# codename0og/codename-rvc-fork-3

Measured on AMD Instinct MI355X. Metric: 48 kHz audio samples/sec end-to-end VC, higher is better.
Workload: dtype f32 (vocoder ResBlock convs and upsamplers, HuBERT, RMVPE's U-Net convs: fp32 operands as exact bf16x3 splits on the bf16 matrix cores -- six products of order <= 2^-16 per multiply-add, fp32 accumulate; everything else fp32 / fp64)

## Files before the change

codename-rvc-fork-3_amd/csrc/decoder.hip:

```cpp
#include <stdlib.h>

#include "decoder.h"

namespace rvc {


constexpr int CARRY_CHUNK = 4096;
__global__ void __launch_bounds__(256)
nsf_carry_kernel(const float *__restrict__ f0, int64_t T, float sr, float upp, float *__restrict__ carry) {
    __shared__ double pre[CARRY_CHUNK];
    __shared__ double part[257];
    __shared__ double cum_s;
    constexpr int SEG = CARRY_CHUNK / 256;
    const int64_t b = blockIdx.x;
    const float *f = f0 + b * T;
    float *c = carry + b * T;
    if (threadIdx.x == 0) {
        c[0] = 0.f;
        cum_s = 0.0;
    }
    for (int64_t base = 0; base + 1 < T; base += CARRY_CHUNK) {
        const int n = (int)((T - 1 - base) < CARRY_CHUNK ? (T - 1 - base) : CARRY_CHUNK);
        for (int i = threadIdx.x; i < n; i += 256) {
            const float last = __fmul_rn(__fdiv_rn(f[base + i], sr), upp);
// ... 409 lines not shown
                if (out->wx.upload(frags)) return 1;
            }
        }
    }
    if (c_in != c_out && !as_bf16 && k >= 7 && winobf_enabled() && winobf_supported(c_in, c_out, k, 1)) {
        std::vector<uint16_t> frags;
        winobf_pack_host(w->data.data(), c_out, c_in, k, &frags);
        if (out->wx.upload(frags)) return 1;
    }
    if (bias) {
        if (need(d, prefix + ".bias", &b, {c_out})) return 1;
        if (out->b.upload(b->data)) return 1;
    }
    out->c_in = c_in; out->c_out = c_out; out->k = k;
    return 0;
}
}

extern "C" int rvc_decoder_create(const rvc_decoder_config *cfg, rvc_decoder **out) {
    if (!cfg || !out) return fail("rvc_decoder_create: null pointer");
    if (cfg->kind != RVC_DEC_NSF && cfg->kind != RVC_DEC_MRF && cfg->kind != RVC_DEC_REFINE)
        return fail("rvc_decoder_create: unknown decoder kind %d", cfg->kind);
    if (cfg->n_ups < 1 || cfg->n_ups > 8) return fail("rvc_decoder_create: n_ups out of range");
    if (cfg->n_res_kernels < 1 || cfg->n_res_kernels > 4 || cfg->n_res_dilations < 1 || cfg->n_res_dilations > 4)
        return fail("rvc_decoder_create: resblock configuration out of range");
    if (cfg->weight_storage != 0 && cfg->weight_storage != 1) return fail("rvc_decoder_create: weight_storage must be 0 (fp32) or 1 (bf16)");
    if (cfg->weight_storage == 1 && cfg->kind == RVC_DEC_REFINE)
        return fail("rvc_decoder_create: bf16 weight storage is built for the NSF / MRF decoders (BASELINE cfg 4), not RefineGAN");
    if (cfg->in_channels % 8 || cfg->upsample_initial_channel % (32 << cfg->n_ups))
        return fail("rvc_decoder_create: channel counts must keep every stage a multiple of 32");
    rvc_decoder *d = new rvc_decoder();
    d->cfg = *cfg;
    d->upp = 1;
    for (int i = 0; i < cfg->n_ups; ++i) d->upp *= cfg->upsample_rates[i];
    if (d->upp > 1024) { delete d; return fail("rvc_decoder_create: prod(upsample_rates) > 1024"); }
    d->dim = cfg->kind == RVC_DEC_MRF ? 9 : 1;
    *out = d;
    return 0;
}

extern "C" int rvc_decoder_set_arithmetic(rvc_decoder *dec, int mode) {
    if (!dec) return fail("rvc_decoder_set_arithmetic: null decoder");
    if (mode != 0 && mode != 1) return fail("rvc_decoder_set_arithmetic: mode must be 0 (exact) or 1 (fp16 pairs), got %d", mode);
    if (dec->finalized) return fail("rvc_decoder_set_arithmetic: decoder already finalized (the tap slabs are packed at finalize)");
    if (mode == 1 && dec->cfg.weight_storage == 1)
        return fail("rvc_decoder_set_arithmetic: fp16 pairs are for fp32 taps; a weight_storage = 1 handle's bf16 taps already cost three products");
    dec->arithmetic = mode;
    return 0;
}

extern "C" int rvc_decoder_set_tensor(rvc_decoder *dec, const char *name, const float *data_host, const int64_t *shape,
                                      int ndim) {
    if (!dec || !name || !data_host || !shape || ndim < 1 || ndim > 4) return fail("rvc_decoder_set_tensor: bad argument");
    if (dec->finalized) return fail("rvc_decoder_set_tensor: decoder already finalized");
    HostTensor t;
    t.shape.assign(shape, shape + ndim);
    const int64_t n = t.numel();
    if (n <= 0) return fail("rvc_decoder_set_tensor: empty tensor '%s'", name);
    t.data.assign(data_host, data_host + n);
    dec->host[name] = std::move(t);
    return 0;
}

extern "C" int rvc_decoder_finalize(rvc_decoder *d) {
    if (!d) return fail("rvc_decoder_finalize: null decoder");
    if (d->finalized) return 0;
    if (d->cfg.kind == RVC_DEC_REFINE) {
        if (refine_finalize(d)) return 1;
        d->host.clear();
        d->finalized = true;
        return 0;
    }
    const rvc_decoder_config &c = d->cfg;
    const bool mrf = c.kind == RVC_DEC_MRF;
    const HostTensor *t;
    if (need(d, "m_source.l_linear.weight", &t, {1, d->dim})) return 1;
    for (int h = 0; h < d->dim; ++h) d->lin_w[h] = t->data[h];
    if (need(d, "m_source.l_linear.bias", &t, {1})) return 1;
    d->lin_b = t->data[0];
    const int c0 = c.upsample_initial_channel;
    if (build_conv(d, "conv_pre", c0, c.in_channels, 7, true, &d->pre)) return 1;
    if (need(d, "cond.weight", &t, {c0, c.gin_channels, 1})) return 1;
    if (d->cond_w.upload(t->data)) return 1;
    if (need(d, "cond.bias", &t, {c0})) return 1;
    if (d->cond_b.upload(t->data)) return 1;
    d->stages.clear();
    d->stages.resize(c.n_ups);
    for (int i = 0; i < c.n_ups; ++i) {
        Stage &s = d->stages[i];
        s.c_in = c0 >> i;
        s.c_out = c0 >> (i + 1);
        s.rate = c.upsample_rates[i];
        s.ksize = c.upsample_kernel_sizes[i];
        s.pad = (s.rate % 2 == 0) ? (s.ksize - s.rate) / 2 : s.rate / 2 + s.rate % 2;
        s.opad = s.rate % 2;
        s.taps = (s.ksize + s.rate - 1) / s.rate;
        if (s.taps > 2) return fail("decoder: upsample kernel %d with rate %d needs %d polyphase taps (max 2)", s.ksize, s.rate, s.taps);
        if (s.taps < 2) s.taps = 2;
        int stride_f0 = 1;
        for (int j = i + 1; j < c.n_ups; ++j) stride_f0 *= c.upsample_rates[j];
        s.nc_stride = stride_f0;
        s.nc_k = stride_f0 == 1 ? 1 : stride_f0 * 2 - stride_f0 % 2;
        s.nc_pad = stride_f0 == 1 ? 0 : (s.nc_k - stride_f0) / 2;
        s.vk = (s.rate - 1) * s.nc_stride + s.nc_k;
        s.vk_rows = (s.vk + 7) / 8 * 8;
        s.S = (int64_t)s.rate * s.nc_stride;
        s.P = (int64_t)s.pad * s.nc_stride + s.nc_pad;
        static const int nc_sep_env = knob("RVC_NC_SEPARATE", 1);
        const bool nc_separate = nc_sep_env && s.vk_rows * 2 >= s.c_in;
        if (nc_separate) {
            s.nc_rows = (s.nc_k + 7) / 8 * 8;
            s.vk = 0;
            s.vk_rows = 0;
        }

        const std::string up = (mrf ? "upsamples." : "ups.") + std::to_string(i);
        const std::string nc = "noise_convs." + std::to_string(i);
        const HostTensor *uw, *ub, *nw, *nb;
        if (need(d, up + ".weight", &uw, {s.c_in, s.c_out, s.ksize})) return 1;
        if (need(d, up + ".bias", &ub, {s.c_out})) return 1;
        if (need(d, nc + ".weight", &nw, {s.c_out, 1, s.nc_k})) return 1;
        if (need(d, nc + ".bias", &nb, {s.c_out})) return 1;
        const int ctot = s.c_in + s.vk_rows;
        const int m_total = s.rate * s.c_out;
        s.interleave = s.rate % 2 == 0;
        auto mrow = [&](int ph, int co) { return s.interleave ? co * s.rate + ph : ph * s.c_out + co; };
        std::vector<float> packed((size_t)s.taps * ctot * m_total, 0.f);
        for (int tp = 0; tp < s.taps; ++tp) {
            const int j = s.taps - 1 - tp;
            for (int ci = 0; ci < s.c_in; ++ci)
                for (int ph = 0; ph < s.rate; ++ph) {
                    const int kk = ph + j * s.rate;
                    if (kk >= s.ksize) continue;
                    for (int co = 0; co < s.c_out; ++co)
                        packed[((size_t)tp * ctot + ci) * m_total + mrow(ph, co)] =
                            uw->data[((size_t)ci * s.c_out + co) * s.ksize + kk];
                }
        }
        const int tp0 = s.taps - 1;
        for (int kq = 0; kq < s.vk; ++kq)
            for (int ph = 0; ph < s.rate; ++ph) {
                const int k = kq - ph * s.nc_stride;
                if (k < 0 || k >= s.nc_k) continue;
                for (int co = 0; co < s.c_out; ++co)
                    packed[((size_t)tp0 * ctot + s.c_in + kq) * m_total + mrow(ph, co)] = nw->data[(size_t)co * s.nc_k + k];
            }
        if (s.w.upload(packed)) return 1;
        std::vector<float> bias(s.c_out);
        for (int co = 0; co < s.c_out; ++co) bias[co] = ub->data[co] + nb->data[co];
        {
            static const int ups_bf = knob("RVC_UPS_BF", 1);
            const int k_n = s.nc_rows > 0 ? 0 : s.nc_k;
            const int vk = upsbf_fold_noise(k_n) ? (s.rate - 1) * s.nc_stride + k_n : 0;
            if (ups_bf && s.opad == 0 && s.rate * s.c_out >= 128 && upsbf_supported(s.c_in, s.c_out, s.rate, s.ksize, vk)) {
                std::vector<uint16_t> frags;
                upsbf_pack_host(uw->data.data(), k_n ? nw->data.data() : nullptr, bias.data(), s.c_in, s.c_out, s.rate, s.ksize, vk, k_n, s.nc_stride, &frags);
                if (s.wub.upload(frags)) return 1;
                s.ub_vk = vk;
            }
        }
        if (s.nc_rows) {
            std::vector<float> ncw((size_t)s.nc_rows * s.c_out, 0.f);
            for (int k = 0; k < s.nc_k; ++k)
                for (int co = 0; co < s.c_out; ++co) ncw[(size_t)k * s.c_out + co] = nw->data[(size_t)co * s.nc_k + k];
            if (s.nc_w.upload(ncw)) return 1;
        }
        if (s.b.upload(bias)) return 1;

        const int nb_ = c.n_res_kernels * c.n_res_dilations;
        s.c1 = std::vector<ConvW>(nb_);
        s.c2 = std::vector<ConvW>(nb_);
        s.pair = std::vector<DevBuf16>(nb_);
        for (int m = 0; m < c.n_res_kernels; ++m)
            for (int j = 0; j < c.n_res_dilations; ++j) {
                std::string p1, p2;
                if (mrf) {
                    const std::string base = "mrfs." + std::to_string(i) + "." + std::to_string(m) + ".layers." + std::to_string(j);
                    p1 = base + ".conv1";
                    p2 = base + ".conv2";
                } else {
                    const std::string base = "resblocks." + std::to_string(i * c.n_res_kernels + m);
                    p1 = base + ".convs1." + std::to_string(j);
                    p2 = base + ".convs2." + std::to_string(j);
                }
                const int k = c.res_kernel_sizes[m];
                const bool b16 = c.weight_storage == 1 && (k == 3 || k == 7 || k == 11);
                if (build_conv(d, p1, s.c_out, s.c_out, k, true, &s.c1[m * c.n_res_dilations + j], b16)) return 1;
                if (build_conv(d, p2, s.c_out, s.c_out, k, true, &s.c2[m * c.n_res_dilations + j], b16)) return 1;
                const int nts = b16 ? 1 : 3;
                if (resblock_bf_enabled() && resblock_bf_supported(s.c_out, k, 1) && resblock_bf_preferred(s.c_out, k, nts)) {
                    const HostTensor *w1, *w2;
                    if (need(d, p1 + ".weight", &w1, {s.c_out, s.c_out, k}) || need(d, p2 + ".weight", &w2, {s.c_out, s.c_out, k})) return 1;
                    std::vector<uint16_t> frags;
                    resblock_bf_pack_host(w1->data.data(), w2->data.data(), s.c_out, k, &frags, nts);
                    s.pair_splits = nts;
                    if (s.pair[m * c.n_res_dilations + j].upload(frags)) return 1;
                }
            }
    }
    d->post_cin = c0 >> c.n_ups;
    if (need(d, "conv_post.weight", &t, {1, d->post_cin, 7})) return 1;
    if (d->post_w.upload(t->data)) return 1;
    d->post_b = 0.f;
    if (mrf) {
        if (need(d, "conv_post.bias", &t, {1})) return 1;
        d->post_b = t->data[0];
    }
    d->host.clear();
    d->finalized = true;
    return 0;
}

extern "C" int rvc_decoder_destroy(rvc_decoder *dec) {
    delete dec;
    return 0;
}

extern "C" int rvc_decoder_upp(const rvc_decoder *dec) { return dec ? dec->upp : 0; }

namespace {
struct Carve {
    size_t off = 0;
    size_t take(size_t bytes) { size_t o = off; off += align_up(bytes, 256); return o; }
};
struct Layout {
    size_t har, carry, biasp, V, p1, p2, wraps, buf[2 + 2 * (MAX_BRANCH_LANES + 1)], total;
    int n_buf;
    int64_t max_cl;
};
constexpr int64_t BRANCH_PARALLEL_MAX_ELEMS = (int64_t)3 * 256 * 128 * 256;
int branch_lanes_wanted(const rvc_decoder *d) {
    const int nk = d->cfg.n_res_kernels, want = d->branch_parallel.load(std::memory_order_relaxed);
    const int most = nk - 1 < MAX_BRANCH_LANES ? nk - 1 : MAX_BRANCH_LANES;
    return want < 0 || want > most ? most : want;
}
Layout make_layout(const rvc_decoder *d, int batch, int64_t T, int64_t Tw) {
    Layout l;
    Carve c;
    const int64_t L = Tw * d->upp;
    l.har = c.take((size_t)batch * L * 4);
    l.carry = c.take((size_t)batch * T * 4);
    l.biasp = c.take((size_t)batch * d->cfg.upsample_initial_channel * 4);
    int64_t len = Tw, max_cl = (int64_t)std::max(d->cfg.upsample_initial_channel, d->cfg.in_channels) * Tw, max_v = 0;
    for (const Stage &s : d->stages) {
        const int64_t nq = len + 1;
        max_v = std::max<int64_t>(max_v, (int64_t)s.vk_rows * nq);
        len = (len - 1) * s.rate - 2 * s.pad + s.ksize + s.opad;
        max_v = std::max<int64_t>(max_v, (int64_t)s.nc_rows * len);
        max_cl = std::max<int64_t>(max_cl, (int64_t)s.c_out * len);
    }
    l.V = c.take((size_t)batch * max_v * 4);
    const size_t scan = d->dim > 1 ? (size_t)batch * d->dim * T : 0;
    l.p1 = c.take(scan * 8);
    l.p2 = c.take(scan * 8);
    l.wraps = c.take(scan * 4);
    l.n_buf = 2 + 2 * (branch_lanes_wanted(d) + 1);
    for (int i = 0; i < l.n_buf; ++i) l.buf[i] = c.take((size_t)batch * max_cl * 4);
    l.total = c.off;
    l.max_cl = max_cl;
    return l;
}
}

extern "C" int rvc_decoder_workspace_bytes(const rvc_decoder *dec, int batch, int64_t n_frames, size_t *bytes) {
    if (!dec || !bytes || batch <= 0 || n_frames <= 0) return fail("rvc_decoder_workspace_bytes: bad argument");
    if (!dec->finalized) return fail("rvc_decoder_workspace_bytes: decoder not finalized");
    *bytes = dec->cfg.kind == RVC_DEC_REFINE ? refine_workspace_bytes(dec, batch, n_frames) : make_layout(dec, batch, n_frames, n_frames).total;
    return 0;
}

extern "C" int rvc_decoder_set_tap(rvc_decoder *dec, int stage, float *tap_dev) {
    if (!dec) return fail("rvc_decoder_set_tap: null decoder");
    dec->tap_stage = tap_dev ? stage : -2;
    dec->tap_dev = tap_dev;
    return 0;
}

int rvc::BranchLanes::create(int n) {
    n_side = n;
    for (int i = 0; i < n; ++i) RVC_HIP(hipStreamCreateWithFlags(&side[i], hipStreamNonBlocking));
    RVC_HIP(hipEventCreateWithFlags(&fork, hipEventDisableTiming));
    for (int i = 0; i <= MAX_BRANCH_LANES; ++i) RVC_HIP(hipEventCreateWithFlags(&last[i], hipEventDisableTiming));
    return 0;
}
rvc::BranchLanes::~BranchLanes() {
    for (int i = 0; i < n_side; ++i) if (side[i]) { (void)hipStreamSynchronize(side[i]); (void)hipStreamDestroy(side[i]); }
    if (fork) (void)hipEventDestroy(fork);
    for (int i = 0; i <= MAX_BRANCH_LANES; ++i) if (last[i]) (void)hipEventDestroy(last[i]);
}

namespace {
int lanes_for(rvc_decoder *d, hipStream_t stream, int n_side, BranchLanes **out) {
    std::lock_guard<std::mutex> g(d->lanes_mu);
    BranchLanes *&l = d->lanes[stream];
    if (l && l->n_side != n_side) { delete l; l = nullptr; }
    if (!l) {
        l = new BranchLanes();
        if (l->create(n_side)) { delete l; l = nullptr; return 1; }
    }
    *out = l;
    return 0;
}
}

extern "C" int rvc_decoder_set_branch_parallel(rvc_decoder *dec, int side_streams) {
    if (!dec) return fail("rvc_decoder_set_branch_parallel: null decoder");
    dec->branch_parallel.store(side_streams, std::memory_order_relaxed);
// ... 292 lines not shown
```

codename-rvc-fork-3_amd/csrc/upsbf.hip:

```cpp
#include <stdlib.h>

#include <algorithm>
#include <mutex>
#include <type_traits>
#include <vector>

#include "conv.h"

namespace rvc {

constexpr int UB_NTH = 512;
constexpr int UB_CK = 64;

struct UbParams {
    const float *x = nullptr;
    const float *har = nullptr;
    const void *u = nullptr;
    const float *bias = nullptr;
    float *y = nullptr;
    int64_t L_in = 0, L_out = 0, Lh = 0;
    int c_in = 0, c_out = 0;
    int n_xchunks = 0;
    int vk = 0;
    int S = 0, P = 0;
    int pad = 0;
    float slope = 0.1f;
    int n_mblk = 0, col_tiles = 0, n_tiles = 0, per_xcd = 0;
};

template <int R, int MB>
struct UbGeom {
    static constexpr int RB_T = MB / 32;
    static constexpr int RBW = RB_T >= 4 ? RB_T / 4 : 1;
    static constexpr int CG = RB_T >= 4 ? 1 : 4 / RB_T;
    static constexpr int N1 = 64 * CG;
    static constexpr int W = N1 * R;
    static constexpr int CPB = (MB - 1) / R + 2;
    static constexpr int KS = UB_CK / 16;
    static constexpr int NGC = 2 * KS;
    static constexpr int PA = 4;
    static constexpr int ROWB = 6 * UB_CK + 16;
    static constexpr int XROWS = N1 + 1;
    static constexpr int X_BYTES = (XROWS + 1) * ROWB;
    static constexpr int RC32 = (XROWS + 31) / 32;
    static constexpr int NIT = (UB_CK / 8) * RC32 / 4;
    static constexpr int IO_FLOATS = CPB * W;
    static constexpr int IO_BYTES = IO_FLOATS * 4 + 16;
    static constexpr int LDS_BYTES = 2 * X_BYTES + IO_BYTES;
    static constexpr int GROUP_BYTES = RB_T * 3 * 1024;
    static_assert(MB == 64 || MB == 128 || MB == 256, "GEMM rows per tile");
    static_assert(R >= 1 && R <= MB, "a channel's phases span at most two m-blocks");
    static_assert((UB_CK / 8) * RC32 % 4 == 0, "the items must divide over the four stager waves");
    static_assert(NGC % PA == 0 && KS % PA == 0, "a chunk's groups must be whole turns of the tap ring");
    static_assert(LDS_BYTES <= 163840, "LDS budget");
};

template <int R, int MB>
__global__ void __launch_bounds__(UB_NTH) __attribute__((amdgpu_waves_per_eu(2, 2)))
upsbf_kernel(const UbParams p) {
    using GM = UbGeom<R, MB>;
    constexpr int RB_T = GM::RB_T, RBW = GM::RBW, N1 = GM::N1, W = GM::W, KS = GM::KS, NGC = GM::NGC, PA = GM::PA, ROWB = GM::ROWB;
    constexpr int NIT = GM::NIT, CK = UB_CK;

    extern __shared__ __attribute__((aligned(16))) unsigned char ub_smem[];
    unsigned char *const xs = ub_smem;
    float *const io_lds = reinterpret_cast<float *>(ub_smem + 2 * GM::X_BYTES);

    const int tid = threadIdx.x, lane = tid & 63;
    const int wave = __builtin_amdgcn_readfirstlane(tid >> 6);
    const int half = lane >> 5, l31 = lane & 31;
    const int64_t L_in = p.L_in, L_out = p.L_out;
    const int nxc = p.n_xchunks, ncht = nxc + (p.vk > 0 ? 1 : 0);
    const int ngt = nxc * NGC + (p.vk > 0 ? KS : 0);
    const int n_mblk = p.n_mblk;
    const int m_total = p.c_out * R;

    const int xcd = blockIdx.x & 7, slot = blockIdx.x >> 3, nslot = gridDim.x >> 3;
    const int tile_end = (xcd + 1) * p.per_xcd < p.n_tiles ? (xcd + 1) * p.per_xcd : p.n_tiles;
    const int tile0 = xcd * p.per_xcd + slot;
    if (tile0 >= tile_end) return;
    const int my_tiles = (tile_end - tile0 + nslot - 1) / nslot;
    const int n_q = my_tiles * ncht;
    auto tile_coords = [&](int tl, int &mblk, int &ct, int &bb) __attribute__((always_inline)) {
        mblk = tl % n_mblk;
        const int rest = tl / n_mblk;
        bb = rest / p.col_tiles;
        ct = rest - bb * p.col_tiles;
    };

    for (int o = tid * 16; o < 2 * GM::X_BYTES; o += UB_NTH * 16) *reinterpret_cast<u32x4 *>(xs + o) = u32x4{0u, 0u, 0u, 0u};
    lds_barrier();
    const int nqp_noise = (p.vk + 1 + 7) / 8;

    if (wave >= 4) {
        __builtin_amdgcn_s_setprio(1);
        const int sw = wave - 4, ht = tid - 256;
        float xr[NIT][4];
        constexpr int RC = GM::RC32;
        const int lq = lane >> 5;
        const unsigned L4 = (unsigned)(L_in * 4);
        const int x_bytes = (int)((int64_t)p.c_in * L_in * 4);
        auto x_issue = [&](int tl, int ci) __attribute__((always_inline)) {
            int mblk, ct, bb;
            tile_coords(tl, mblk, ct, bb);
            const int q0m1 = ct * N1 - 1;
            int sw_o = sw;
            asm volatile("" : "+s"(sw_o));
            if (ci < nxc) {
                const __amdgpu_buffer_rsrc_t rs = __builtin_amdgcn_make_buffer_rsrc((void *)(p.x + (int64_t)bb * p.c_in * L_in), 0, x_bytes, RSRC_RAW32);
                const unsigned Lu = (unsigned)L_in;
                const int ch0 = ci * CK;
#pragma unroll
                for (int i = 0; i < NIT; ++i) {
                    const int wi = sw_o * NIT + i, qp = wi / RC, rc = wi - qp * RC;
                    const int qd = 2 * qp + lq, r = rc * 32 + l31;
                    const unsigned tg = (unsigned)(q0m1 + r);
                    const bool ok = r < GM::XROWS && tg < Lu;
                    const unsigned base = (unsigned)(ch0 + 4 * qd) * L4 + tg * 4u;
#pragma unroll
                    for (int e = 0; e < 4; ++e)
                        xr[i][e] = __builtin_bit_cast(float, __builtin_amdgcn_raw_buffer_load_b32(rs, (int)(ok ? base + (unsigned)e * L4 : BUF_OOB), 0, 0));
                }
            } else {
                const int h_bytes = (int)(p.Lh * 4);
                const __amdgpu_buffer_rsrc_t rs = __builtin_amdgcn_make_buffer_rsrc((void *)(p.har + (int64_t)bb * p.Lh), 0, h_bytes, RSRC_RAW32);
                const int vk = p.vk;
#pragma unroll
                for (int i = 0; i < NIT; ++i) {
                    const int wi = sw_o * NIT + i, qp = wi / RC, rc = wi - qp * RC;
                    if (qp >= nqp_noise) continue;
                    const int qd = 2 * qp + lq, r = rc * 32 + l31;
                    const int q = q0m1 + r;
                    const bool okq = r < GM::XROWS && q >= 0 && q <= (int)L_in;
                    const int64_t idx0 = (int64_t)q * p.S - p.P + 4 * qd;
#pragma unroll
                    for (int e = 0; e < 4; ++e) {
                        const int64_t idx = idx0 + e;
                        const bool ok = okq && 4 * qd + e < vk && idx >= 0 && idx < p.Lh;
                        xr[i][e] = __builtin_bit_cast(float, __builtin_amdgcn_raw_buffer_load_b32(rs, (int)(ok ? (unsigned)idx * 4u : BUF_OOB), 0, 0));
                        if (4 * qd + e == vk) xr[i][e] = 1.f;
                    }
                }
            }
        };
        auto x_write = [&](int q, int ci) __attribute__((always_inline)) {
            unsigned char *const xb = xs + (q & 1) * GM::X_BYTES;
            const float slope = ci < nxc ? p.slope : 1.f;
            int sw_o = sw;
            asm volatile("" : "+s"(sw_o));
#pragma unroll
            for (int i = 0; i < NIT; ++i) {
                const int wi = sw_o * NIT + i, qp = wi / RC, rc = wi - qp * RC;
                if (ci >= nxc && qp >= nqp_noise) continue;
                const int qd = 2 * qp + lq, r = rc * 32 + l31;
                unsigned w[2][3];
#pragma unroll
                for (int e2 = 0; e2 < 2; ++e2) {
                    const float va = xr[i][2 * e2], vb = xr[i][2 * e2 + 1];
                    split3_np(__builtin_fmaxf(va, mul_np(va, slope)), __builtin_fmaxf(vb, mul_np(vb, slope)), w[e2]);
                }
                unsigned char *o = xb + (r < GM::XROWS ? r : GM::XROWS) * ROWB + qd * 8;
#pragma unroll
                for (int s = 0; s < 3; ++s) *reinterpret_cast<u32x2 *>(o + s * 2 * CK) = u32x2{w[0][s], w[1][s]};
                if (i & 1) __builtin_amdgcn_sched_barrier(0);
            }
        };
        const int y_bytes = (int)((int64_t)p.c_out * L_out * 4);
        const bool fold = p.vk > 0;
        auto out_store = [&](int tl) __attribute__((always_inline)) {
            int mblk, ct, bb;
            tile_coords(tl, mblk, ct, bb);
            const __amdgpu_buffer_rsrc_t yrs = __builtin_amdgcn_make_buffer_rsrc((void *)(p.y + (int64_t)bb * p.c_out * L_out), 0, y_bytes, RSRC_RAW32);
            const int64_t t_base = (int64_t)ct * N1 * R - p.pad;
            const int m0 = mblk * MB, co0 = m0 / R;
            constexpr int n_el = GM::CPB * W;
            const unsigned Lo4 = (unsigned)(L_out * 4);
            for (int f0 = 0; f0 < n_el; f0 += 4 * 256) {
                float v[4], bv[4];
                unsigned off[4];
#pragma unroll
                for (int k = 0; k < 4; ++k) {
                    const int f = f0 + k * 256 + ht;
                    const int row = f / W, i = f - row * W;
                    const int64_t t = t_base + i;
                    const int m = (co0 + row) * R + i % R;
                    const bool ok = f < n_el && m >= m0 && m < m0 + MB && m < m_total && t >= 0 && t < L_out;
                    v[k] = io_lds[f < n_el ? f : 0];
                    bv[k] = !fold && p.bias && ok ? p.bias[co0 + row] : 0.f;
                    off[k] = ok ? (unsigned)(co0 + row) * Lo4 + (unsigned)t * 4u : BUF_OOB;
                }
#pragma unroll
                for (int k = 0; k < 4; ++k) __builtin_amdgcn_raw_buffer_store_b32(__builtin_bit_cast(unsigned, v[k] + bv[k]), yrs, (int)off[k], 0, 0);
            }
        };
        int wt = 0, wc = 0, it = 0, ic = 0;
        auto adv = [&](int &t_, int &c_) __attribute__((always_inline)) {
            if (++c_ == ncht) { c_ = 0; ++t_; }
        };
        x_issue(tile0, 0);
        x_write(0, 0);
        adv(wt, wc); adv(it, ic);
        if (1 < n_q) x_issue(tile0 + it * nslot, ic);
        adv(it, ic);
        int ct_i = 0, cc_i = 0;
        for (int q = 0; q < n_q; ++q) {
            lds_barrier();
            if (cc_i == 0 && q > 0) out_store(tile0 + (ct_i - 1) * nslot);
            if (ncht == 1) lds_barrier();
            if (q + 1 < n_q) x_write(q + 1, wc);
            adv(wt, wc);
            asm volatile("s_waitcnt vmcnt(8)" ::: "memory");
            if (q + 2 < n_q) x_issue(tile0 + it * nslot, ic);
            adv(it, ic);
            adv(ct_i, cc_i);
        }
        lds_barrier();
        out_store(tile0 + (my_tiles - 1) * nslot);
        return;
    }

    const int rb0 = RB_T >= 4 ? RBW * wave : wave % RB_T;
    const int col0 = RB_T >= 4 ? 0 : 64 * (wave / RB_T);
    const __amdgpu_buffer_rsrc_t urs = __builtin_amdgcn_make_buffer_rsrc((void *)p.u, 0, n_mblk * ngt * GM::GROUP_BYTES, RSRC_RAW32);
    bf16x8 fa[PA][RBW][3];
    bf16x8 fb[2][2][3];
    f32x16 acc[RBW][2];
    auto load_a1 = [&](int slot_a, int byte_off, int rb, int s) __attribute__((always_inline)) {
        fa[slot_a][rb][s] = __builtin_bit_cast(bf16x8, __builtin_amdgcn_raw_buffer_load_b128(urs, 16 * lane + ((rb0 + rb) * 3 + s) * 1024, byte_off, 0));
    };
    auto load_b1 = [&](int buf, const unsigned char *src, int gc, int cb, int s) __attribute__((always_inline)) {
        const int j = gc / KS, ks = gc - j * KS;
        fb[buf][cb][s] = __builtin_bit_cast(bf16x8, *reinterpret_cast<const u32x4 *>(src + (1 - j) * ROWB + ks * 32 + cb * 32 * ROWB + s * 2 * CK));
    };
    const int x_lane = (col0 + l31) * ROWB + half * 16;
    constexpr int ia6[6] = {0, 1, 0, 2, 1, 0}, ib6[6] = {2, 1, 1, 0, 0, 0};
    constexpr int NM = 12 * RBW;

    int mblk, ct, bb;
    tile_coords(tile0, mblk, ct, bb);
    int a_base = mblk * ngt * GM::GROUP_BYTES;
#pragma unroll
    for (int g = 0; g < PA - 1; ++g)
#pragma unroll
        for (int rb = 0; rb < RBW; ++rb)
#pragma unroll
            for (int s = 0; s < 3; ++s) load_a1(g, a_base + g * GM::GROUP_BYTES, rb, s);

    int q = 0;
    for (int t = 0; t < my_tiles; ++t) {
        const int tl = tile0 + t * nslot;
        tile_coords(tl, mblk, ct, bb);
        a_base = mblk * ngt * GM::GROUP_BYTES;
        int a_next = a_base;
        if (t + 1 < my_tiles) {
            int m2, c2, b2;
            tile_coords(tl + nslot, m2, c2, b2);
            a_next = m2 * ngt * GM::GROUP_BYTES;
        }
#pragma unroll
        for (int rb = 0; rb < RBW; ++rb)
#pragma unroll
            for (int cb = 0; cb < 2; ++cb)
#pragma unroll
                for (int r = 0; r < 16; ++r) acc[rb][cb][r] = 0.f;
        int g0 = 0;
#pragma unroll 1
        for (int c = 0; c < ncht; ++c, ++q) {
            const bool noise = c == nxc;
            lds_barrier();
            const unsigned char *const src = xs + (q & 1) * GM::X_BYTES + x_lane;
#pragma unroll
            for (int k = 0; k < 6; ++k) load_b1(0, src, 0, k & 1, 2 - (k >> 1));
#pragma unroll
            for (int gc = 0; gc < NGC; ++gc) {
                if (gc >= KS && noise) break;
                const int nlast = noise ? KS : NGC;
#pragma unroll
                for (int i = 0; i < 6; ++i)
#pragma unroll
                    for (int cb = 0; cb < 2; ++cb)
#pragma unroll
                        for (int rb = 0; rb < RBW; ++rb) {
                            const int k = (2 * i + cb) * RBW + rb;
                            acc[rb][cb] = __builtin_amdgcn_mfma_f32_32x32x16_bf16(fa[gc % PA][rb][ia6[i]], fb[gc & 1][cb][ib6[i]], acc[rb][cb], 0, 0, 0);
                            __builtin_amdgcn_sched_barrier(0);
                            if (k < 6 && gc + 1 < nlast) load_b1((gc + 1) & 1, src, gc + 1, k & 1, 2 - (k >> 1));
                            if (k >= NM - 3 * RBW) {
                                const int kk = k - (NM - 3 * RBW);
                                int gn = g0 + gc + PA - 1;
                                const int off = gn >= ngt ? a_next + (gn - ngt) * GM::GROUP_BYTES : a_base + gn * GM::GROUP_BYTES;
                                load_a1((gc + PA - 1) % PA, off, kk / 3, kk % 3);
                            }
                            __builtin_amdgcn_sched_barrier(0);
                        }
            }
            g0 += noise ? KS : NGC;
        }
        if (ncht == 1) lds_barrier();
#pragma unroll
        for (int rb = 0; rb < RBW; ++rb)
#pragma unroll
            for (int r = 0; r < 16; ++r) {
                const int m = mblk * MB + 32 * (rb0 + rb) + (r & 3) + 8 * (r >> 2) + 4 * half;
                const int co = m / R, ph = m - co * R;
                const int co_l = co - (mblk * MB) / R;
                if (m < m_total) {
                    float *const o = io_lds + co_l * W + (col0 + l31) * R + ph;
                    o[0] = acc[rb][0][r];
                    o[32 * R] = acc[rb][1][r];
                }
            }
    }
    lds_barrier();
}


static int ub_mb(int rate, int c_out) {
    const int64_t rows = (int64_t)rate * c_out;
    return rows >= 256 ? 256 : rows >= 128 ? 128 : 64;
}

bool upsbf_supported(int c_in, int c_out, int rate, int ksize, int vk) {
    if (!(rate == 2 || rate == 8 || rate == 10 || rate == 12)) return false;
    if (c_in % UB_CK || c_in < UB_CK || c_out < 1 || ksize > 2 * rate || ksize < rate) return false;
    if (vk < 0 || vk >= UB_CK) return false;
    return rate == 2 || ub_mb(rate, c_out) >= 128;
}

static void ub_dims(int c_in, int c_out, int rate, int vk, int *mb, int *n_mblk, int *ngt) {
    *mb = ub_mb(rate, c_out);
    *n_mblk = (rate * c_out + *mb - 1) / *mb;
    *ngt = (c_in / UB_CK) * 8 + (vk > 0 ? 4 : 0);
}

size_t upsbf_weight_bytes(int c_in, int c_out, int rate, int vk) {
    int mb, n_mblk, ngt;
    ub_dims(c_in, c_out, rate, vk, &mb, &n_mblk, &ngt);
    return (size_t)n_mblk * ngt * (mb / 32) * 3 * 1024;
}

void upsbf_pack_host(const float *uw, const float *nw, const float *bias, int c_in, int c_out, int rate, int ksize, int vk, int nc_k,
                     int nc_stride, std::vector<uint16_t> *out) {
    int mb, n_mblk, ngt;
    ub_dims(c_in, c_out, rate, vk, &mb, &n_mblk, &ngt);
    const int RB_T = mb / 32, nxc = c_in / UB_CK;
    out->assign(upsbf_weight_bytes(c_in, c_out, rate, vk) / 2, 0);
    auto put = [&](size_t group, int rb, int lane, int e, float v) {
        uint16_t h[3];
        bf16_split_host(v, 3, h);
        for (int s = 0; s < 3; ++s) (*out)[((group * RB_T + rb) * 3 + s) * 512 + lane * 8 + e] = h[s];
    };
    for (int mblk = 0; mblk < n_mblk; ++mblk)
        for (int rb = 0; rb < RB_T; ++rb)
            for (int lane = 0; lane < 64; ++lane) {
                const int m = mblk * mb + 32 * rb + (lane & 31);
                const int co = m / rate, ph = m % rate;
                const bool row_ok = co < c_out;
                for (int c = 0; c < nxc; ++c)
                    for (int j = 0; j < 2; ++j)
                        for (int ks = 0; ks < 4; ++ks)
                            for (int e = 0; e < 8; ++e) {
                                const int ci = UB_CK * c + 16 * ks + 8 * (lane >> 5) + e;
                                const int kk = ph + j * rate;
                                const float v = row_ok && kk < ksize ? uw[((size_t)ci * c_out + co) * ksize + kk] : 0.f;
                                put((size_t)mblk * ngt + c * 8 + j * 4 + ks, rb, lane, e, v);
                            }
                if (vk > 0)
                    for (int ks = 0; ks < 4; ++ks)
                        for (int e = 0; e < 8; ++e) {
                            const int kq = 16 * ks + 8 * (lane >> 5) + e;
                            const int k = kq - ph * nc_stride;
                            float v = row_ok && kq < vk && k >= 0 && k < nc_k ? nw[(size_t)co * nc_k + k] : 0.f;
                            if (row_ok && kq == vk && bias) v = bias[co];
                            put((size_t)mblk * ngt + nxc * 8 + ks, rb, lane, e, v);
                        }
            }
}

template <int R, int MB>
static int ub_launch(UbParams p, int batch, hipStream_t stream) {
    using GM = UbGeom<R, MB>;
    if (reserve_whole_cu((const void *)upsbf_kernel<R, MB>, "upsbf")) return 1;
    p.col_tiles = (int)ceil_div(p.L_in + 1, GM::N1);
    p.n_tiles = p.col_tiles * p.n_mblk * batch;
    const PersistentGrid g = persistent_grid(p.n_tiles);
    p.per_xcd = g.per_xcd;
    hipLaunchKernelGGL((upsbf_kernel<R, MB>), dim3(g.blocks), dim3(UB_NTH), LDS_WHOLE_CU, stream, p);
    RVC_LAUNCH_CHECK();
    return 0;
}

int launch_upsbf(const float *x, const float *har, int64_t Lh, const void *u, const float *bias, float *y, int batch, int c_in, int c_out,
                 int64_t L_in, int64_t L_out, int rate, int ksize, int pad, int vk, int64_t S, int64_t P, float slope, hipStream_t stream) {
    if (!upsbf_supported(c_in, c_out, rate, ksize, vk)) return fail("upsbf: unsupported shape (%d -> %d channels, rate %d, kernel %d, %d noise rows)", c_in, c_out, rate, ksize, vk);
    if (vk > 0 && (!har || Lh <= 0 || !fits_2gib(Lh, 4) || S > 4096 || P > 65536)) return fail("upsbf: bad noise source");
    if (!fits_2gib((int64_t)c_in * L_in, 4) || !fits_2gib((int64_t)c_out * L_out, 4)) return fail("upsbf: slab exceeds the 2 GiB buffer addressing");
    if (L_in <= 0 || batch <= 0) return 0;
    UbParams p;
    p.x = x; p.har = har; p.u = u; p.bias = bias; p.y = y; p.L_in = L_in; p.L_out = L_out; p.Lh = vk > 0 ? Lh : 0;
    p.c_in = c_in; p.c_out = c_out; p.n_xchunks = c_in / UB_CK; p.vk = vk; p.S = (int)S; p.P = (int)P; p.pad = pad; p.slope = slope;
    int mb, ngt;
    ub_dims(c_in, c_out, rate, vk, &mb, &p.n_mblk, &ngt);
#define RVC_UB_CASE(RR, MM) if (rate == RR && mb == MM) return ub_launch<RR, MM>(p, batch, stream)
    RVC_UB_CASE(12, 256); RVC_UB_CASE(10, 256); RVC_UB_CASE(8, 256);
    RVC_UB_CASE(12, 128); RVC_UB_CASE(10, 128); RVC_UB_CASE(8, 128);
    RVC_UB_CASE(2, 256); RVC_UB_CASE(2, 128); RVC_UB_CASE(2, 64);
#undef RVC_UB_CASE
    return fail("upsbf: no instantiation for rate %d with %d GEMM rows per tile", rate, mb);
}

bool upsbf_fold_noise(int nc_k) { return nc_k > 0; }

}

using namespace rvc;

extern "C" int rvc_upsample_bf16x3_weight_bytes(int c_in, int c_out, int rate, int ksize, int nc_k, int nc_stride, size_t *bytes) {
    if (!bytes) return fail("rvc_upsample_bf16x3_weight_bytes: null pointer");
    if (nc_k < 0 || (nc_k > 0 && nc_stride < 1)) return fail("rvc_upsample_bf16x3_weight_bytes: bad noise conv (%d taps, stride %d)", nc_k, nc_stride);
    const int vk = upsbf_fold_noise(nc_k) ? (rate - 1) * nc_stride + nc_k : 0;
    if (!upsbf_supported(c_in, c_out, rate, ksize, vk))
        return fail("rvc_upsample_bf16x3_weight_bytes: unsupported shape (%d -> %d channels, rate %d, kernel %d, %d noise rows): rate must be 2, "
                    "8, 10 or 12 (8 / 10 / 12 with rate * c_out >= 128), c_in a multiple of 64, rate <= ksize <= 2 rate, "
                    "(rate - 1) nc_stride + nc_k <= 63", c_in, c_out, rate, ksize, vk);
    *bytes = upsbf_weight_bytes(c_in, c_out, rate, vk);
    return 0;
}

extern "C" int rvc_upsample_bf16x3_pack_weight(const float *up_w_host, const float *noise_w_host, const float *bias_host, int c_in, int c_out,
                                               int rate, int ksize, int nc_k, int nc_stride, void *u_dev, void *stream) {
    if (!up_w_host || !u_dev || (nc_k > 0 && !noise_w_host)) return fail("rvc_upsample_bf16x3_pack_weight: null pointer");
    size_t bytes = 0;
    if (rvc_upsample_bf16x3_weight_bytes(c_in, c_out, rate, ksize, nc_k, nc_stride, &bytes)) return 1;
    const int vk = upsbf_fold_noise(nc_k) ? (rate - 1) * nc_stride + nc_k : 0;
    std::vector<uint16_t> u;
    upsbf_pack_host(up_w_host, noise_w_host, bias_host, c_in, c_out, rate, ksize, vk, nc_k, nc_stride, &u);
    return upload_packed("rvc_upsample_bf16x3_pack_weight", u.data(), bytes, u_dev, stream);
}

extern "C" int rvc_upsample_bf16x3_forward(const float *x_dev, const float *har_dev, int64_t har_len, const void *u_dev, const float *bias_dev,
                                           float *y_dev, int batch, int c_in, int c_out, int64_t length_in, int rate, int ksize, int pad,
                                           int nc_k, int nc_stride, int nc_pad, float slope_in, void *stream) {
    if (!x_dev || !u_dev || !y_dev) return fail("rvc_upsample_bf16x3_forward: null pointer");
    if (pad < 0 || nc_k < 0 || (nc_k > 0 && nc_stride < 1)) return fail("rvc_upsample_bf16x3_forward: bad argument");
    const int vk = upsbf_fold_noise(nc_k) ? (rate - 1) * nc_stride + nc_k : 0;
    const int64_t l_out = (length_in - 1) * rate - 2 * pad + ksize;
    if (l_out <= 0) return fail("rvc_upsample_bf16x3_forward: empty output");
    return launch_upsbf(x_dev, har_dev, har_len, u_dev, bias_dev, y_dev, batch, c_in, c_out, length_in, l_out, rate, ksize, pad, vk,
                        (int64_t)rate * nc_stride, (int64_t)pad * nc_stride + nc_pad, slope_in, (hipStream_t)stream);
}
```

Baseline: 63.17 million.

## Vectorize upsampler output stores, move store after staging, split halo load

The upsampler's output store now writes 128-bit buffer stores from a padded, alignment-shifted LDS tile, falling back to per-element stores only at edges. The store is moved after the next chunk's input staging and issue, so it overlaps with loads, and explicit vmcnt waits bound how many memory operations are in flight. The halo row is loaded separately by one wave, which simplifies row indexing, and the noise index math is tightened. The gate now also sends small layers (rate*c_out < 128) to the bf16x3 path unless the knob is 2, and debug cycle-stamp instrumentation is added under a compile flag. The hand-tuned waitcnt values carry a risk of hazards, and the wider gate sends small layers through a kernel that was previously skipped for them.

```diff
diff --git a/codename-rvc-fork-3_amd/csrc/decoder.hip b/codename-rvc-fork-3_amd/csrc/decoder.hip
--- a/codename-rvc-fork-3_amd/csrc/decoder.hip
+++ b/codename-rvc-fork-3_amd/csrc/decoder.hip
@@ -585,7 +585,7 @@
             static const int ups_bf = knob("RVC_UPS_BF", 1);
             const int k_n = s.nc_rows > 0 ? 0 : s.nc_k;
             const int vk = upsbf_fold_noise(k_n) ? (s.rate - 1) * s.nc_stride + k_n : 0;
-            if (ups_bf && s.opad == 0 && s.rate * s.c_out >= 128 && upsbf_supported(s.c_in, s.c_out, s.rate, s.ksize, vk)) {
+            if (ups_bf && s.opad == 0 && (s.rate * s.c_out >= 128 || ups_bf != 2) && upsbf_supported(s.c_in, s.c_out, s.rate, s.ksize, vk)) {
                 std::vector<uint16_t> frags;
                 upsbf_pack_host(uw->data.data(), k_n ? nw->data.data() : nullptr, bias.data(), s.c_in, s.c_out, s.rate, s.ksize, vk, k_n, s.nc_stride, &frags);
                 if (s.wub.upload(frags)) return 1;
diff --git a/codename-rvc-fork-3_amd/csrc/upsbf.hip b/codename-rvc-fork-3_amd/csrc/upsbf.hip
--- a/codename-rvc-fork-3_amd/csrc/upsbf.hip
+++ b/codename-rvc-fork-3_amd/csrc/upsbf.hip
@@ -26,6 +26,7 @@
     int pad = 0;
     float slope = 0.1f;
     int n_mblk = 0, col_tiles = 0, n_tiles = 0, per_xcd = 0;
+    unsigned long long *stamps = nullptr;
 };
 
 template <int R, int MB>
@@ -41,10 +42,11 @@
     static constexpr int PA = 4;
     static constexpr int ROWB = 6 * UB_CK + 16;
     static constexpr int XROWS = N1 + 1;
-    static constexpr int X_BYTES = (XROWS + 1) * ROWB;
-    static constexpr int RC32 = (XROWS + 31) / 32;
+    static constexpr int X_BYTES = XROWS * ROWB;
+    static constexpr int RC32 = N1 / 32;
     static constexpr int NIT = (UB_CK / 8) * RC32 / 4;
-    static constexpr int IO_FLOATS = CPB * W;
+    static constexpr int WS = W + 4;
+    static constexpr int IO_FLOATS = CPB * WS;
     static constexpr int IO_BYTES = IO_FLOATS * 4 + 16;
     static constexpr int LDS_BYTES = 2 * X_BYTES + IO_BYTES;
     static constexpr int GROUP_BYTES = RB_T * 3 * 1024;
@@ -52,10 +54,12 @@
     static_assert(R >= 1 && R <= MB, "a channel's phases span at most two m-blocks");
     static_assert((UB_CK / 8) * RC32 % 4 == 0, "the items must divide over the four stager waves");
     static_assert(NGC % PA == 0 && KS % PA == 0, "a chunk's groups must be whole turns of the tap ring");
+    static_assert(4 * NIT + 1 + 8 <= 56, "memory operations in flight per stager wave: a chunk's loads, the halo's, and the stores the loop leaves pending");
     static_assert(LDS_BYTES <= 163840, "LDS budget");
 };
 
-template <int R, int MB>
+constexpr int UB_STAMP_CHUNKS = 16;
+template <int R, int MB, int DBG = 0>
 __global__ void __launch_bounds__(UB_NTH) __attribute__((amdgpu_waves_per_eu(2, 2)))
 upsbf_kernel(const UbParams p) {
     using GM = UbGeom<R, MB>;
@@ -91,11 +95,21 @@
     for (int o = tid * 16; o < 2 * GM::X_BYTES; o += UB_NTH * 16) *reinterpret_cast<u32x4 *>(xs + o) = u32x4{0u, 0u, 0u, 0u};
     lds_barrier();
     const int nqp_noise = (p.vk + 1 + 7) / 8;
+    const int ish = (4 - (p.pad & 3)) & 3;
+    unsigned long long *const stamps = (DBG & 128) ? p.stamps + ((size_t)blockIdx.x * 2 + (wave >= 4 ? 1 : 0)) * (UB_STAMP_CHUNKS * 8) : nullptr;
+    auto stamp = [&](int chunk, int k) __attribute__((always_inline)) {
+        if constexpr (DBG & 128) {
+            __builtin_amdgcn_sched_barrier(0);
+            if ((wave == 0 || wave == 4) && lane == 0 && chunk < UB_STAMP_CHUNKS) stamps[chunk * 8 + k] = __builtin_readcyclecounter();
+            __builtin_amdgcn_sched_barrier(0);
+        }
+    };
 
     if (wave >= 4) {
         __builtin_amdgcn_s_setprio(1);
         const int sw = wave - 4, ht = tid - 256;
         float xr[NIT][4];
+        float xh = 0.f;
         constexpr int RC = GM::RC32;
         const int lq = lane >> 5;
         const unsigned L4 = (unsigned)(L_in * 4);
@@ -113,13 +127,16 @@
 #pragma unroll
                 for (int i = 0; i < NIT; ++i) {
                     const int wi = sw_o * NIT + i, qp = wi / RC, rc = wi - qp * RC;
-                    const int qd = 2 * qp + lq, r = rc * 32 + l31;
+                    const int qd = 2 * qp + lq, r = 1 + rc * 32 + l31;
                     const unsigned tg = (unsigned)(q0m1 + r);
-                    const bool ok = r < GM::XROWS && tg < Lu;
-                    const unsigned base = (unsigned)(ch0 + 4 * qd) * L4 + tg * 4u;
+                    const unsigned off = tg < Lu ? (unsigned)(ch0 + 4 * qd) * L4 + tg * 4u : BUF_OOB;
 #pragma unroll
                     for (int e = 0; e < 4; ++e)
-                        xr[i][e] = __builtin_bit_cast(float, __builtin_amdgcn_raw_buffer_load_b32(rs, (int)(ok ? base + (unsigned)e * L4 : BUF_OOB), 0, 0));
+                        xr[i][e] = __builtin_bit_cast(float, __builtin_amdgcn_raw_buffer_load_b32(rs, (int)off, e * (int)L4, 0));
+                }
+                if (sw_o == 3) {
+                    const unsigned tg = (unsigned)q0m1;
+                    xh = __builtin_bit_cast(float, __builtin_amdgcn_raw_buffer_load_b32(rs, (int)(tg < Lu ? (unsigned)(ch0 + lane) * L4 + tg * 4u : BUF_OOB), 0, 0));
                 }
             } else {
                 const int h_bytes = (int)(p.Lh * 4);
@@ -129,16 +146,17 @@
                 for (int i = 0; i < NIT; ++i) {
                     const int wi = sw_o * NIT + i, qp = wi / RC, rc = wi - qp * RC;
                     if (qp >= nqp_noise) continue;
-                    const int qd = 2 * qp + lq, r = rc * 32 + l31;
+                    const int qd = 2 * qp + lq, r = 1 + rc * 32 + l31;
                     const int q = q0m1 + r;
-                    const bool okq = r < GM::XROWS && q >= 0 && q <= (int)L_in;
                     const int64_t idx0 = (int64_t)q * p.S - p.P + 4 * qd;
+                    const bool near = (q <= (int)L_in) & (idx0 > -4) & (idx0 < p.Lh);
+                    const int i0 = near ? (int)idx0 : -4;
+                    const unsigned Lhu = (unsigned)p.Lh;
 #pragma unroll
                     for (int e = 0; e < 4; ++e) {
-                        const int64_t idx = idx0 + e;
-                        const bool ok = okq && 4 * qd + e < vk && idx >= 0 && idx < p.Lh;
-                        xr[i][e] = __builtin_bit_cast(float, __builtin_amdgcn_raw_buffer_load_b32(rs, (int)(ok ? (unsigned)idx * 4u : BUF_OOB), 0, 0));
-                        if (4 * qd + e == vk) xr[i][e] = 1.f;
+                        const unsigned idx = (unsigned)(i0 + e);
+                        const bool ok = (4 * qd + e < vk) & (idx < Lhu);
+                        xr[i][e] = __builtin_bit_cast(float, __builtin_amdgcn_raw_buffer_load_b32(rs, (int)(ok ? idx * 4u : BUF_OOB), 0, 0));
                     }
                 }
             }
@@ -152,46 +170,92 @@
             for (int i = 0; i < NIT; ++i) {
                 const int wi = sw_o * NIT + i, qp = wi / RC, rc = wi - qp * RC;
                 if (ci >= nxc && qp >= nqp_noise) continue;
-                const int qd = 2 * qp + lq, r = rc * 32 + l31;
+                const int qd = 2 * qp + lq, r = 1 + rc * 32 + l31;
+                if (ci >= nxc) {
+#pragma unroll
+                    for (int e = 0; e < 4; ++e)
+                        if (4 * qd + e == p.vk) xr[i][e] = 1.f;
+                }
                 unsigned w[2][3];
 #pragma unroll
                 for (int e2 = 0; e2 < 2; ++e2) {
                     const float va = xr[i][2 * e2], vb = xr[i][2 * e2 + 1];
                     split3_np(__builtin_fmaxf(va, mul_np(va, slope)), __builtin_fmaxf(vb, mul_np(vb, slope)), w[e2]);
                 }
-                unsigned char *o = xb + (r < GM::XROWS ? r : GM::XROWS) * ROWB + qd * 8;
+                unsigned char *o = xb + r * ROWB + qd * 8;
 #pragma unroll
                 for (int s = 0; s < 3; ++s) *reinterpret_cast<u32x2 *>(o + s * 2 * CK) = u32x2{w[0][s], w[1][s]};
                 if (i & 1) __builtin_amdgcn_sched_barrier(0);
+            }
+            if (ci < nxc && sw_o == 3) {
+                unsigned w[3];
+                split3_np(__builtin_fmaxf(xh, mul_np(xh, slope)), 0.f, w);
+#pragma unroll
+                for (int s = 0; s < 3; ++s) *reinterpret_cast<unsigned short *>(xb + s * 2 * CK + lane * 2) = (unsigned short)w[s];
             }
         };
         const int y_bytes = (int)((int64_t)p.c_out * L_out * 4);
         const bool fold = p.vk > 0;
-        auto out_store = [&](int tl) __attribute__((always_inline)) {
+        const bool al4 = (L_out & 3) == 0 && (reinterpret_cast<uintptr_t>(p.y) & 15) == 0;
+        auto out_store_as = [&](int tl, auto with_bias) __attribute__((always_inline)) {
+            constexpr bool WB = decltype(with_bias)::value;
+            constexpr int WS = GM::WS, VPR = WS / 4, VM = VPR - 2, CPB = GM::CPB;
             int mblk, ct, bb;
             tile_coords(tl, mblk, ct, bb);
             const __amdgpu_buffer_rsrc_t yrs = __builtin_amdgcn_make_buffer_rsrc((void *)(p.y + (int64_t)bb * p.c_out * L_out), 0, y_bytes, RSRC_RAW32);
-            const int64_t t_base = (int64_t)ct * N1 * R - p.pad;
+            const int t_col0 = ct * W - p.pad - ish;
             const int m0 = mblk * MB, co0 = m0 / R;
-            constexpr int n_el = GM::CPB * W;
+            const int m_end = m0 + MB < m_total ? m0 + MB : m_total;
             const unsigned Lo4 = (unsigned)(L_out * 4);
-            for (int f0 = 0; f0 < n_el; f0 += 4 * 256) {
-                float v[4], bv[4];
-                unsigned off[4];
+            const int Lo = (int)L_out;
+            auto put = [&](int row, int jv, bool live, f32x4 v, float b) __attribute__((always_inline)) {
+                const int i0 = 4 * jv - ish, t0 = t_col0 + 4 * jv, ch = co0 + row;
+                const int mlo = m0 - ch * R, mhi = m_end - ch * R;
+                const unsigned o = (unsigned)ch * Lo4 + (unsigned)t0 * 4u;
+                const bool whole = live & al4 & (mlo <= 0) & (mhi >= R) & (i0 >= 0) & (i0 + 3 < W) & (t0 >= 0) & (t0 + 3 < Lo);
+                const float r[4] = {v.x + b, v.y + b, v.z + b, v.w + b};
+                asm volatile("s_waitcnt vmcnt(51)" ::: "memory");
+                __builtin_amdgcn_raw_buffer_store_b128(__builtin_bit_cast(u32x4, f32x4{r[0], r[1], r[2], r[3]}), yrs, (int)(whole ? o : BUF_OOB), 0, 0);
+                if (live & !whole) {
+                    int ph = (i0 + 4 * R) % R;
+                    asm volatile("s_waitcnt vmcnt(48)" ::: "memory");
+#pragma unroll
+                    for (int e = 0; e < 4; ++e) {
+                        const bool ok = (i0 + e >= 0) & (i0 + e < W) & (t0 + e >= 0) & (t0 + e < Lo) & (ph >= mlo) & (ph < mhi);
+                        __builtin_amdgcn_raw_buffer_store_b32(__builtin_bit_cast(unsigned, r[e]), yrs, (int)(ok ? o + 4u * (unsigned)e : BUF_OOB), 0, 0);
+                        ph = ph + 1 == R ? 0 : ph + 1;
+                    }
+                }
+            };
+            auto bias_of = [&](int row, bool live) __attribute__((always_inline)) {
+                if constexpr (WB) return live && co0 + row < p.c_out ? p.bias[co0 + row] : 0.f;
+                else return 0.f;
+            };
+            constexpr int n_main = CPB * VM;
+            for (int f0 = 0; f0 < n_main; f0 += 4 * 256) {
+                f32x4 v[4];
+                float bv[4];
+                int row[4], jv[4];
 #pragma unroll
                 for (int k = 0; k < 4; ++k) {
                     const int f = f0 + k * 256 + ht;
-                    const int row = f / W, i = f - row * W;
-                    const int64_t t = t_base + i;
-                    const int m = (co0 + row) * R + i % R;
-                    const bool ok = f < n_el && m >= m0 && m < m0 + MB && m < m_total && t >= 0 && t < L_out;
-                    v[k] = io_lds[f < n_el ? f : 0];
-                    bv[k] = !fold && p.bias && ok ? p.bias[co0 + row] : 0.f;
-                    off[k] = ok ? (unsigned)(co0 + row) * Lo4 + (unsigned)t * 4u : BUF_OOB;
-                }
-#pragma unroll
-                for (int k = 0; k < 4; ++k) __builtin_amdgcn_raw_buffer_store_b32(__builtin_bit_cast(unsigned, v[k] + bv[k]), yrs, (int)off[k], 0, 0);
-            }
+                    row[k] = f < n_main ? f / VM : 0;
+                    jv[k] = f < n_main ? 1 + f - row[k] * VM : 1;
+                    v[k] = *reinterpret_cast<const f32x4 *>(io_lds + row[k] * WS + 4 * jv[k]);
+                    bv[k] = bias_of(row[k], f < n_main);
+                }
+#pragma unroll
+                for (int k = 0; k < 4; ++k) put(row[k], jv[k], f0 + k * 256 + ht < n_main, v[k], bv[k]);
+            }
+            for (int f0 = 0; f0 < 2 * CPB; f0 += 256) {
+                const int f = f0 + ht;
+                const int row = f < 2 * CPB ? f >> 1 : 0, jv = (f & 1) ? VPR - 1 : 0;
+                put(row, jv, f < 2 * CPB, *reinterpret_cast<const f32x4 *>(io_lds + row * WS + 4 * jv), bias_of(row, f < 2 * CPB));
+            }
+        };
+        auto out_store = [&](int tl) __attribute__((always_inline)) {
+            if (!fold && p.bias) out_store_as(tl, std::true_type{});
+            else out_store_as(tl, std::false_type{});
         };
         int wt = 0, wc = 0, it = 0, ic = 0;
         auto adv = [&](int &t_, int &c_) __attribute__((always_inline)) {
@@ -204,14 +268,21 @@
         adv(it, ic);
         int ct_i = 0, cc_i = 0;
         for (int q = 0; q < n_q; ++q) {
+            stamp(q, 0);
             lds_barrier();
-            if (cc_i == 0 && q > 0) out_store(tile0 + (ct_i - 1) * nslot);
-            if (ncht == 1) lds_barrier();
+            stamp(q, 1);
+            if constexpr (DBG & 128) asm volatile("s_waitcnt vmcnt(0)" ::: "memory");
+            stamp(q, 2);
             if (q + 1 < n_q) x_write(q + 1, wc);
+            stamp(q, 3);
             adv(wt, wc);
             asm volatile("s_waitcnt vmcnt(8)" ::: "memory");
             if (q + 2 < n_q) x_issue(tile0 + it * nslot, ic);
+            stamp(q, 4);
             adv(it, ic);
+            if (cc_i == 0 && q > 0) out_store(tile0 + (ct_i - 1) * nslot);
+            if (ncht == 1) lds_barrier();
+            stamp(q, 5);
             adv(ct_i, cc_i);
         }
         lds_barrier();
@@ -267,7 +338,9 @@
 #pragma unroll 1
         for (int c = 0; c < ncht; ++c, ++q) {
             const bool noise = c == nxc;
+            stamp(q, 0);
             lds_barrier();
+            stamp(q, 1);
             const unsigned char *const src = xs + (q & 1) * GM::X_BYTES + x_lane;
 #pragma unroll
             for (int k = 0; k < 6; ++k) load_b1(0, src, 0, k & 1, 2 - (k >> 1));
@@ -305,7 +378,7 @@
                 const int co = m / R, ph = m - co * R;
                 const int co_l = co - (mblk * MB) / R;
                 if (m < m_total) {
-                    float *const o = io_lds + co_l * W + (col0 + l31) * R + ph;
+                    float *const o = io_lds + co_l * GM::WS + ish + (col0 + l31) * R + ph;
                     o[0] = acc[rb][0][r];
                     o[32 * R] = acc[rb][1][r];
                 }
@@ -377,15 +450,15 @@
             }
 }
 
-template <int R, int MB>
+template <int R, int MB, int DBG = 0>
 static int ub_launch(UbParams p, int batch, hipStream_t stream) {
     using GM = UbGeom<R, MB>;
-    if (reserve_whole_cu((const void *)upsbf_kernel<R, MB>, "upsbf")) return 1;
+    if (reserve_whole_cu((const void *)upsbf_kernel<R, MB, DBG>, "upsbf")) return 1;
     p.col_tiles = (int)ceil_div(p.L_in + 1, GM::N1);
     p.n_tiles = p.col_tiles * p.n_mblk * batch;
     const PersistentGrid g = persistent_grid(p.n_tiles);
     p.per_xcd = g.per_xcd;
-    hipLaunchKernelGGL((upsbf_kernel<R, MB>), dim3(g.blocks), dim3(UB_NTH), LDS_WHOLE_CU, stream, p);
+    hipLaunchKernelGGL((upsbf_kernel<R, MB, DBG>), dim3(g.blocks), dim3(UB_NTH), LDS_WHOLE_CU, stream, p);
     RVC_LAUNCH_CHECK();
     return 0;
 }
@@ -401,6 +474,13 @@
     p.c_in = c_in; p.c_out = c_out; p.n_xchunks = c_in / UB_CK; p.vk = vk; p.S = (int)S; p.P = (int)P; p.pad = pad; p.slope = slope;
     int mb, ngt;
     ub_dims(c_in, c_out, rate, vk, &mb, &p.n_mblk, &ngt);
+#ifdef RVC_ABLATE
+    static const int dbg = knob("RVC_UB_DBG", 0);
+    p.stamps = reinterpret_cast<unsigned long long *>(const_cast<float *>(vk > 0 ? bias : har));
+#define RVC_UB_DBG_CASE(RR, MM) if (dbg == 128 && p.stamps && rate == RR && mb == MM) return ub_launch<RR, MM, 128>(p, batch, stream)
+    RVC_UB_DBG_CASE(12, 256); RVC_UB_DBG_CASE(10, 256); RVC_UB_DBG_CASE(2, 128); RVC_UB_DBG_CASE(2, 64);
+#undef RVC_UB_DBG_CASE
+#endif
 #define RVC_UB_CASE(RR, MM) if (rate == RR && mb == MM) return ub_launch<RR, MM>(p, batch, stream)
     RVC_UB_CASE(12, 256); RVC_UB_CASE(10, 256); RVC_UB_CASE(8, 256);
     RVC_UB_CASE(12, 128); RVC_UB_CASE(10, 128); RVC_UB_CASE(8, 128);
```

Measured after the change: 61.67 million. -2.4%, worse.
